# remydubois/illico

Hardware: NVIDIA B200
Metric: gene_x_group_tests_per_s (higher is better)
Workload: dtype f32 keys / int64 ranks / f64 epilogue

## Files before the change

illico_b200/csrc/fused.cu:

```cuda
#include "common.cuh"
#include "epilogue.cuh"
#include "tma.cuh"

#include <stdlib.h>

namespace illico {

int launch_stage_dense_list(const float* X, long long ld, int gene_lb, const int* list, const int* n_list_dev, const int* mode_dev,
                            int want_mode, const illico_plan_t* plan, float* ir_vals, uint32_t* ir_cnt, cudaStream_t stream);
int launch_stage_dense_tma_if(const float* X, long long ld, int gene_lb, int b, const illico_plan_t* plan, float* ir_vals,
                              uint32_t* ir_cnt, int seg_lo, int seg_hi, cudaStream_t stream, int segs_per_cta_req,
                              const int* mode_dev, int want_mode);
int launch_stage_csr_if(const float*, const int32_t*, const long long*, int, int, const illico_plan_t*, float*, uint32_t*, void*, size_t,
                        const int*, int, cudaStream_t);
int launch_stage_csr_list(const float*, const int32_t*, const long long*, int, int, const int*, const int*, int, int,
                          const illico_plan_t*, float*, uint32_t*, cudaStream_t);
int launch_ovo_mapped(const float*, const uint32_t*, int, const int*, const int*, int, const illico_plan_t*, const illico_flags_t*, double*,
                      long long, void*, size_t, const illico_debug_t*, cudaStream_t);
int launch_ovr_mapped(const float*, const uint32_t*, int, const int*, const int*, int, const illico_plan_t*, const illico_flags_t*, double*,
                      long long, void*, size_t, const illico_debug_t*, cudaStream_t);
bool stage_dense_tma_ok(const float* X, long long ld, int gene_lb, int b, const illico_plan_t* plan);
int launch_stage_dense_tma(const float* X, long long ld, int gene_lb, int b, const illico_plan_t* plan, float* ir_vals,
                           uint32_t* ir_cnt, int seg_lo, int seg_hi, cudaStream_t stream, int segs_per_cta = 0);

// ... 23 lines not shown
    double* gc;
    int Gs;
};
constexpr int DW = 64;
constexpr int CLS_NARROW = 1, CLS_IDENT = 2, CLS_WANTS_WIDE = 4;
constexpr int WIDE_FROM = 11;
constexpr int HB_NONE = 0, HB_LIST = 1, HB_ALL = 2;
constexpr int GC_MU = 0, GC_NRNT = 1, GC_PROD12 = 2, GC_DENOM = 3, GC_INV_NT = 4, GC_N = 5;

size_t gtab_bytes(int b, int G) {
    const size_t bs = (size_t)((b + 63) & ~63), Gs = (size_t)((G + 63) & ~63);
    return bs * ((size_t)DCAP * 20 + 4 + 8 + 8 + 1 + 8 + 2 + (size_t)DW * 2) + Gs * 8 * GC_N + 1024;
}
Gtab gtab_carve(void* ws, int b, int G) {
    const size_t bs = (size_t)((b + 63) & ~63), Gs = (size_t)((G + 63) & ~63);
    char* p = reinterpret_cast<char*>((reinterpret_cast<uintptr_t>(ws) + 255) & ~(uintptr_t)255);
    Gtab c;
    c.Gs = (int)Gs;
    c.gc = reinterpret_cast<double*>(p); p += Gs * 8 * GC_N;
    c.fval = reinterpret_cast<double*>(p); p += bs * 8 * DCAP;
    c.tie = reinterpret_cast<unsigned long long*>(p); p += bs * 8;
    c.sum = reinterpret_cast<double*>(p); p += bs * 8;
    c.key = reinterpret_cast<float*>(p); p += bs * 4 * DCAP;
    c.mult = reinterpret_cast<uint32_t*>(p); p += bs * 4 * DCAP;
    c.wgt = reinterpret_cast<uint32_t*>(p); p += bs * 4 * DCAP;
    c.nnz = reinterpret_cast<uint32_t*>(p); p += bs * 4;
    c.n_bad = reinterpret_cast<int*>(p); p += 64;
    c.list = reinterpret_cast<int*>(p); p += bs * 4;
    c.cmap = reinterpret_cast<int*>(p); p += bs * 4;
    c.wm = reinterpret_cast<uint32_t*>(p); p += bs * 2 * DW;
    c.bad = reinterpret_cast<unsigned char*>(p); p += bs;
    c.cls = reinterpret_cast<unsigned char*>(p); p += bs;
    c.mode = reinterpret_cast<unsigned char*>(p);
    return c;
}

constexpr float ROUND_MAGIC = 12582912.0f;
constexpr uint32_t ROUND_MAGIC_BITS = 0x4B400000u;
__device__ __forceinline__ uint32_t count_bin(float v, bool& ok) {
    const float tt = __fadd_rn(v, ROUND_MAGIC);
    const uint32_t q1 = __float_as_uint(tt) - (ROUND_MAGIC_BITS + 1u);
    ok = (__fsub_rn(tt, ROUND_MAGIC) == v) && (q1 < (uint32_t)DW);
    return q1;
}

__global__ void __launch_bounds__(256) fused_ctab_kernel(const float* __restrict__ ir_vals, const uint32_t* __restrict__ ir_cnt,
                                                         int b, const illico_plan_t pl, int seg_lo, int seg_hi, int is_log1p,
                                                         Gtab gt, int bs, int wide_on) {
    __shared__ uint32_t wh[8][DW];
    const int lane = threadIdx.x & 31, wl = threadIdx.x >> 5;
    const int warp = (blockIdx.x * blockDim.x + threadIdx.x) >> 5, nwarps = (gridDim.x * blockDim.x) >> 5;
    const int S = pl.n_segments;
    for (int j = warp; j < b; j += nwarps) {
        float mykey = 0.0f;
        uint32_t mycnt = 0;
        int D = 0;
        bool nbad = false;
        bool general = false;
        for (int s = seg_lo; s < seg_hi && !nbad; ++s) {
            const int c = (int)ir_cnt[(long long)j * S + s];
            const float* src = ir_vals + (long long)j * pl.slot_cap + pl.seg_base[s];
            for (int i0 = 0; i0 < c && !nbad; i0 += 32) {
                const bool valid = i0 + lane < c;
                const float v = valid ? src[i0 + lane] : 0.0f;
                if (__any_sync(FULL, valid && !(v > 0.0f))) { nbad = general = true; break; }
                const unsigned same = __match_any_sync(FULL, __float_as_uint(v));
                const bool leader = valid && (__ffs(same) - 1 == lane);
                const uint32_t n = (uint32_t)__popc(same);
                unsigned leaders = __ballot_sync(FULL, leader);
                while (leaders) {
                    const int l = __ffs(leaders) - 1;
                    leaders &= leaders - 1;
                    const float vv = __shfl_sync(FULL, v, l);
                    const uint32_t nn = __shfl_sync(FULL, n, l);
                    const unsigned hit = __ballot_sync(FULL, lane < D && mykey == vv);
                    if (hit) {
                        if (lane == __ffs(hit) - 1) mycnt += nn;
                    } else if (D < DCAP) {
                        if (lane == D) { mykey = vv; mycnt = nn; }
                        ++D;
                    } else {
                        nbad = true;
                        break;
                    }
                }
            }
        }
        bool ident = wide_on != 0 && !general;
        if (ident) {
            wh[wl][lane] = 0u;
            wh[wl][lane + 32] = 0u;
            __syncwarp();
            if (!nbad) {
                bool okv = true;
                const uint32_t q1 = count_bin(mykey, okv);
                if (__any_sync(FULL, lane < D && !okv)) ident = false;
                else if (lane < D) wh[wl][q1] = mycnt;
            } else {
                for (int s = seg_lo; s < seg_hi && ident; ++s) {
                    const int c = (int)ir_cnt[(long long)j * S + s];
                    const float* src = ir_vals + (long long)j * pl.slot_cap + pl.seg_base[s];
                    for (int i0 = 0; i0 < c; i0 += 32) {
                        const bool valid = i0 + lane < c;
                        const float v = valid ? src[i0 + lane] : 0.0f;
                        bool okv;
                        const uint32_t q1 = count_bin(v, okv);
                        if (__any_sync(FULL, valid && !okv)) { ident = false; break; }
                        const unsigned same = __match_any_sync(FULL, __float_as_uint(v));
                        if (valid && (__ffs(same) - 1 == lane)) wh[wl][q1] += (uint32_t)__popc(same);
                        __syncwarp();
                    }
                }
            }
            __syncwarp();
        }
        int cls = nbad ? 0 : CLS_NARROW;
        if (ident) {
            const uint32_t c0 = wh[wl][lane], c1 = wh[wl][lane + 32];
            if (__any_sync(FULL, (c0 | c1) > 0xffffu)) {
                ident = false;
            } else {
                const uint32_t e0 = wh[wl][2 * lane], e1 = wh[wl][2 * lane + 1];
                gt.wm[(long long)lane * bs + j] = e0 | (e1 << 16);
                cls |= CLS_IDENT;
                if (nbad || D >= WIDE_FROM) cls |= CLS_WANTS_WIDE;
            }
        }
        __syncwarp();
        if (lane == 0) gt.cls[j] = (unsigned char)cls;
        if (nbad) continue;
        int pos = 0;
        for (int t = 0; t < D; ++t) pos += (__shfl_sync(FULL, mykey, t) < mykey) ? 1 : 0;
        const bool mine = lane < D;
        if (mine) { gt.key[(long long)pos * bs + j] = mykey; gt.mult[(long long)pos * bs + j] = mycnt; }
        if (lane >= D && lane < DCAP) { gt.key[(long long)lane * bs + j] = 0.0f; gt.mult[(long long)lane * bs + j] = 0u; }
        const uint32_t nnz = warp_sum<uint32_t>(mine ? mycnt : 0u);
        const unsigned long long tie = warp_sum_u64(mine ? (unsigned long long)cube_minus((long long)mycnt) : 0ull);
        const double sum = warp_sum_f64(mine ? (double)mycnt * fc_value(mykey, is_log1p) : 0.0);
        if (lane == 0) { gt.nnz[j] = nnz; gt.tie[j] = tie; gt.sum[j] = sum; }
    }
}

__global__ void __launch_bounds__(256) fused_mode_kernel(int b, Gtab gt) {
    const int j = blockIdx.x * blockDim.x + threadIdx.x;
    const int c = (j < b) ? gt.cls[j] : 0;
    const bool tile_wide = __syncthreads_or((c & CLS_WANTS_WIDE) != 0) != 0;
    const int mode = (tile_wide && (c & CLS_IDENT)) ? 1 : 0;
    const bool bad = j < b && mode == 0 && !(c & CLS_NARROW);
    if (j < b) { gt.mode[j] = (unsigned char)mode; gt.bad[j] = bad ? 1 : 0; }
    const int nb = __syncthreads_count(bad);
    if (threadIdx.x == 0 && nb) atomicAdd(gt.n_bad, nb);
}

template <int ROWS, int STAGES, int BUF>
struct FusedLayout {
    static constexpr int ROW_BYTES = FUSED_LANES * 4;
    static constexpr int STAGE_BYTES = ROWS * ROW_BYTES;
    static constexpr int RING_OFF = 0;
    static constexpr int NZ_OFF = STAGES * STAGE_BYTES;
    static constexpr int KEY_OFF = NZ_OFF + BUF * ROW_BYTES;
    static constexpr int HIST_OFF = KEY_OFF + DCAP * ROW_BYTES;
    static constexpr int BAR_OFF = HIST_OFF + DCAP * FUSED_LANES * 2;
    static constexpr int BYTES = BAR_OFF + 2 * STAGES * 8;
};

template <int ROWS, int STAGES, int BUF, int MINB, bool OVO>
__global__ void __launch_bounds__(FUSED_THREADS, MINB) fused_pass_kernel(const float* __restrict__ X, long long ld, int gene_lb,
                                                                         int b, const illico_plan_t pl, int groups_per_cta,
                                                                         Gtab gt, int bs, unsigned long long* __restrict__ rec,
                                                                         long long gstride, int share_1024) {
    using L = FusedLayout<ROWS, STAGES, BUF>;
    static_assert(32 % ROWS == 0 && BUF > ROWS, "layout");
    extern __shared__ __align__(128) unsigned char smem[];
    const uint32_t smem_a = (uint32_t)__cvta_generic_to_shared(smem);
    const uint32_t bars = smem_a + L::BAR_OFF;
    const int t = threadIdx.x, lane = t & 31, w = t >> 5;
    const int G = pl.n_groups, ref = OVO ? pl.ref_group : -1;
    const int gy0 = blockIdx.y * groups_per_cta, gy1 = min(G, gy0 + groups_per_cta);
    const int p_begin = pl.seg_pos[pl.group_seg[gy0]], p_end = pl.seg_pos[pl.group_seg[gy1]];
    const bool ref_in = ref >= gy0 && ref < gy1;
    const int ref_p0 = ref_in ? pl.seg_pos[pl.group_seg[ref]] : 0;
    const int ref_len = ref_in ? pl.seg_pos[pl.group_seg[ref + 1]] - ref_p0 : 0;
    const int nv = p_end - p_begin - ref_len;
    const int g0 = blockIdx.x * FUSED_LANES;
    const uint32_t row_bytes = (uint32_t)min(FUSED_LANES, (b - g0 + 3) & ~3) * 4u;
    if (nv <= 0) return;
    if ((long long)gt.n_bad[0] * 1024 > (long long)b * share_1024) return;
    if (__syncthreads_and(t >= FUSED_LANES || g0 + t >= b || gt.bad[g0 + t] != 0 || gt.mode[g0 + t] != 0)) return;

    if (t == 0) {
        for (int i = 0; i < STAGES; ++i) {
            mbar_init(bars + 8 * i, 1);
            mbar_init(bars + 8 * (STAGES + i), FUSED_WARPS);
        }
        asm volatile("fence.mbarrier_init.release.cluster;" ::: "memory");
    }
    __syncthreads();

    if (w == FUSED_WARPS) {
        uint64_t policy;
        asm volatile("createpolicy.fractional.L2::evict_first.b64 %0, 1.0;" : "=l"(policy));
        const char* base = reinterpret_cast<const char*>(X + gene_lb + g0);
        const unsigned long long ldb = (unsigned long long)ld * 4ull;
        auto row_of = [&](int i) {
            int p = p_begin + i;
            if (ref_in && p >= ref_p0) p += ref_len;
            return pl.perm[p];
        };
        int myrow = (lane < nv) ? row_of(lane) : 0;
        int k = 0;
        for (int i0 = 0; i0 < nv; i0 += 32) {
            const int nxt = (i0 + 32 + lane < nv) ? row_of(i0 + 32 + lane) : 0;
            const int nrows = min(32, nv - i0);
#pragma unroll
            for (int q = 0; q < 32 / ROWS; ++q, ++k) {
                if (q * ROWS >= nrows) break;
                const int slot = k % STAGES;
                const uint32_t full = bars + 8 * slot, empty = bars + 8 * (STAGES + slot);
                mbar_wait(empty, ((k / STAGES) & 1) ^ 1);
                const int rows_here = min(ROWS, nrows - q * ROWS);
                if (lane == 0) mbar_expect_tx(full, (uint32_t)rows_here * row_bytes);
                __syncwarp();
                const int u = lane - q * ROWS;
                if (u >= 0 && u < rows_here)
                    bulk_g2s(smem_a + L::RING_OFF + slot * L::STAGE_BYTES + u * L::ROW_BYTES,
                             base + (unsigned long long)(uint32_t)myrow * ldb, row_bytes, full, policy);
            }
            myrow = nxt;
        }
        return;
    }

    const int j = g0 + t;
    const bool in_batch = j < b;
    const uint32_t keys_a = smem_a + L::KEY_OFF + t * 4;
    const uint32_t hist_a = smem_a + L::HIST_OFF + t * 2;
    const uint32_t nz_a = smem_a + L::NZ_OFF + t * 4;
    auto lds_f = [](uint32_t a) { float v; asm volatile("ld.shared.f32 %0, [%1];" : "=f"(v) : "r"(a)); return v; };
    auto sts_f = [](uint32_t a, float v) { asm volatile("st.shared.f32 [%0], %1;" ::"r"(a), "f"(v) : "memory"); };
    auto lds_h = [](uint32_t a) { uint16_t v; asm volatile("ld.shared.u16 %0, [%1];" : "=h"(v) : "r"(a)); return (uint32_t)v; };
    auto sts_h = [](uint32_t a, uint32_t v) { asm volatile("st.shared.u16 [%0], %1;" ::"r"(a), "h"((uint16_t)v) : "memory"); };
    const bool mine = in_batch && gt.bad[j] == 0 && gt.mode[j] == 0;
    bool bad = !mine;
    float* gkey = gt.key + (in_batch ? j : 0);
    int D = 0;
#pragma unroll
    for (int q = 0; q < DCAP; ++q) {
        const float kq = bad ? 0.0f : __ldcg(gkey + (long long)q * bs);
        if (kq != 0.0f) D = q + 1;
        sts_f(keys_a + q * L::ROW_BYTES, kq);
        sts_h(hist_a + q * (FUSED_LANES * 2), 0u);
    }
    uint32_t Hacc[OVO ? 1 : DCAP];
#pragma unroll
    for (int q = 0; q < (OVO ? 1 : DCAP); ++q) Hacc[q] = 0u;
    uint32_t wr = nz_a;

    auto drain = [&]() {
        const uint32_t mywr = bad ? nz_a : wr;
        const uint32_t maxwr = __reduce_max_sync(FULL, mywr - nz_a);
        for (uint32_t o = 0; o < maxwr; o += L::ROW_BYTES) {
            if (nz_a + o < mywr) {
                const float v = lds_f(nz_a + o);
                int q = (int)v - 1;
                if (!(q >= 0 && q < D && lds_f(keys_a + q * L::ROW_BYTES) == v)) {
                    q = 0;
                    while (q < D && lds_f(keys_a + q * L::ROW_BYTES) != v) ++q;
                    if (q == D) {
                        int slot = -1;
                        if (v > 0.0f) {
                            for (int r = D; r < DCAP && slot < 0; ++r) {
                                const unsigned old = atomicCAS(reinterpret_cast<unsigned*>(gkey + (long long)r * bs), 0u,
                                                               __float_as_uint(v));
                                const float kv = old ? __uint_as_float(old) : v;
                                sts_f(keys_a + r * L::ROW_BYTES, kv);
                                D = r + 1;
                                if (kv == v) slot = r;
                            }
                        }
                        if (slot < 0) { bad = true; q = 0; }
                        else q = slot;
                    }
                }
                const uint32_t ha = hist_a + q * (FUSED_LANES * 2);
                sts_h(ha, lds_h(ha) + 1u);
            }
        }
        wr = nz_a;
    };
    auto close_group = [&](int g) {
        drain();
        unsigned long long wds[3] = {0ull, 0ull, 0ull};
#pragma unroll
        for (int q = 0; q < DCAP; ++q) {
            const uint32_t bq = lds_h(hist_a + q * (FUSED_LANES * 2));
            wds[q >> 2] |= (unsigned long long)bq << (16 * (q & 3));
            if (!OVO) Hacc[OVO ? 0 : q] += bq;
            sts_h(hist_a + q * (FUSED_LANES * 2), 0u);
        }
        if (!bad) {
            unsigned long long* o = rec + (long long)g * gstride + (long long)j * 3;
            o[0] = wds[0]; o[1] = wds[1]; o[2] = wds[2];
        }
    };
    auto group_end_v = [&](int gg) { return pl.seg_pos[pl.group_seg[gg + 1]] - p_begin - ((ref_in && gg > ref) ? ref_len : 0); };
    int g = (gy0 == ref) ? gy0 + 1 : gy0;
    int gend = group_end_v(g);

    auto append = [&](float v) {
        asm volatile("{ .reg .pred p; setp.neu.f32 p, %1, 0f00000000; @p st.shared.f32 [%0], %1; @p add.u32 %0, %0, %2; }"
                     : "+r"(wr)
                     : "f"(v), "n"(L::ROW_BYTES)
                     : "memory");
    };
    const uint32_t ring_a = smem_a + L::RING_OFF + t * 4;
    const uint32_t wr_limit = nz_a + (uint32_t)(BUF - ROWS) * L::ROW_BYTES;
    int slot = 0;
    uint32_t parity = 0;
    for (int i = 0; i < nv; i += ROWS) {
        mbar_wait(bars + 8 * slot, parity);
        const uint32_t src = ring_a + slot * L::STAGE_BYTES;
        if (i + ROWS <= gend) {
            float v[ROWS];
#pragma unroll
            for (int u = 0; u < ROWS; ++u) v[u] = lds_f(src + u * L::ROW_BYTES);
#pragma unroll
            for (int u = 0; u < ROWS; ++u) append(v[u]);
        } else {
            const int nr = min(ROWS, nv - i);
#pragma unroll 1
            for (int u = 0; u < nr; ++u) {
                if (i + u == gend) {
                    close_group(g);
                    ++g;
                    if (g == ref) ++g;
                    gend = group_end_v(g);
                }
                append(lds_f(src + u * L::ROW_BYTES));
            }
        }
        __syncwarp();
        if (lane == 0) mbar_arrive(bars + 8 * (STAGES + slot));
        if (++slot == STAGES) { slot = 0; parity ^= 1u; }
        if (__any_sync(FULL, wr > wr_limit)) drain();
    }
    close_group(g);
    if (mine) {
        if (bad) {
            gt.bad[j] = 1;
        } else if (!OVO) {
#pragma unroll
            for (int q = 0; q < (OVO ? 1 : DCAP); ++q)
                if (Hacc[q]) atomicAdd(gt.mult + (long long)q * bs + j, Hacc[q]);
        }
    }
}

template <int ROWS, int STAGES>
struct WideLayout {
    static constexpr int ROW_BYTES = FUSED_LANES * 4;
    static constexpr int STAGE_BYTES = ROWS * ROW_BYTES;
    static constexpr int RING_OFF = 0;
    static constexpr int HIST_OFF = STAGES * STAGE_BYTES;
    static constexpr int ATAB_OFF = HIST_OFF + (DW / 2) * ROW_BYTES;
    static constexpr int BAR_OFF = ATAB_OFF + (DW / 2) * ROW_BYTES;
    static constexpr int BYTES = BAR_OFF + 2 * STAGES * 8;
};
constexpr int WIDE_M_SHIFT = 40;
static_assert(DW % 2 == 0 && DW <= 64, "packed layout: two 16-bit bins per word; the table step keeps two bins per lane");

template <int ROWS, int STAGES, int MINB>
__global__ void __launch_bounds__(FUSED_THREADS, MINB) fused_wide_pass_kernel(const float* __restrict__ X, long long ld, int gene_lb,
                                                                              int b, const illico_plan_t pl, int groups_per_cta,
                                                                              Gtab gt, int bs, unsigned long long* __restrict__ rec,
                                                                              long long gstride, int share_1024) {
    using L = WideLayout<ROWS, STAGES>;
    static_assert(32 % ROWS == 0, "layout");
    extern __shared__ __align__(128) unsigned char smem[];
    const uint32_t smem_a = (uint32_t)__cvta_generic_to_shared(smem);
    const uint32_t bars = smem_a + L::BAR_OFF;
    const int t = threadIdx.x, lane = t & 31, w = t >> 5;
    const int G = pl.n_groups, ref = pl.ref_group;
    const int g0 = blockIdx.x * FUSED_LANES;
    const uint32_t row_bytes = (uint32_t)min(FUSED_LANES, (b - g0 + 3) & ~3) * 4u;
    if ((long long)gt.n_bad[0] * 1024 > (long long)b * share_1024) return;
    if (__syncthreads_and(t >= FUSED_LANES || g0 + t >= b || gt.bad[g0 + t] != 0 || gt.mode[g0 + t] != 1)) return;

    if (t == 0) {
        for (int i = 0; i < STAGES; ++i) {
            mbar_init(bars + 8 * i, 1);
            mbar_init(bars + 8 * (STAGES + i), FUSED_WARPS);
        }
        asm volatile("fence.mbarrier_init.release.cluster;" ::: "memory");
    }
    __syncthreads();
    const int n_chunks = (G + groups_per_cta - 1) / groups_per_cta;
    struct Chunk { int gy0, p_begin, ref_p0, ref_len, nv; bool ref_in; };
    auto chunk_of = [&](int c) {
        Chunk k;
        k.gy0 = c * groups_per_cta;
        const int gy1 = min(G, k.gy0 + groups_per_cta);
        k.p_begin = pl.seg_pos[pl.group_seg[k.gy0]];
        const int p_end = pl.seg_pos[pl.group_seg[gy1]];
        k.ref_in = ref >= k.gy0 && ref < gy1;
        k.ref_p0 = k.ref_in ? pl.seg_pos[pl.group_seg[ref]] : 0;
        k.ref_len = k.ref_in ? pl.seg_pos[pl.group_seg[ref + 1]] - k.ref_p0 : 0;
        k.nv = p_end - k.p_begin - k.ref_len;
        return k;
    };

    if (w == FUSED_WARPS) {
        uint64_t policy;
        asm volatile("createpolicy.fractional.L2::evict_first.b64 %0, 1.0;" : "=l"(policy));
        const char* base = reinterpret_cast<const char*>(X + gene_lb + g0);
        const unsigned long long ldb = (unsigned long long)ld * 4ull;
        int k = 0;
        for (int c = blockIdx.y; c < n_chunks; c += gridDim.y) {
            const Chunk ch = chunk_of(c);
            auto row_of = [&](int i) {
                int p = ch.p_begin + i;
                if (ch.ref_in && p >= ch.ref_p0) p += ch.ref_len;
                return pl.perm[p];
            };
            int myrow = (lane < ch.nv) ? row_of(lane) : 0;
            for (int i0 = 0; i0 < ch.nv; i0 += 32) {
                const int nxt = (i0 + 32 + lane < ch.nv) ? row_of(i0 + 32 + lane) : 0;
                const int nrows = min(32, ch.nv - i0);
#pragma unroll
                for (int q = 0; q < 32 / ROWS; ++q, ++k) {
                    if (q * ROWS >= nrows) break;
                    const int slot = k % STAGES;
                    const uint32_t full = bars + 8 * slot, empty = bars + 8 * (STAGES + slot);
                    mbar_wait_backoff(empty, ((k / STAGES) & 1) ^ 1);
                    const int rows_here = min(ROWS, nrows - q * ROWS);
                    if (lane == 0) mbar_expect_tx(full, (uint32_t)rows_here * row_bytes);
                    __syncwarp();
                    const int u = lane - q * ROWS;
                    if (u >= 0 && u < rows_here)
                        bulk_g2s(smem_a + L::RING_OFF + slot * L::STAGE_BYTES + u * L::ROW_BYTES,
                                 base + (unsigned long long)(uint32_t)myrow * ldb, row_bytes, full, policy);
                }
                myrow = nxt;
            }
        }
        return;
    }

    const int j = g0 + t;
    const bool in_batch = j < b;
    const bool mine = in_batch && gt.bad[j] == 0 && gt.mode[j] == 1;
    const uint32_t hist_a = smem_a + L::HIST_OFF + (uint32_t)(w >> 1) * 128u + (uint32_t)lane * 4u + (uint32_t)(w & 1) * 2u;
    const uint32_t atab_a = smem_a + L::ATAB_OFF + t * 4;
    constexpr uint32_t BIN_BYTES = FUSED_LANES * 2;
    auto lds_f = [](uint32_t a) { float v; asm volatile("ld.shared.f32 %0, [%1];" : "=f"(v) : "r"(a)); return v; };
    auto lds_u = [](uint32_t a) { uint32_t v; asm volatile("ld.shared.u32 %0, [%1];" : "=r"(v) : "r"(a) : "memory"); return v; };
    auto sts_u = [](uint32_t a, uint32_t v) { asm volatile("st.shared.u32 [%0], %1;" ::"r"(a), "r"(v) : "memory"); };
    auto lds_h = [](uint32_t a) { uint32_t v; asm volatile("ld.shared.u16 %0, [%1];" : "=r"(v) : "r"(a) : "memory"); return v; };
    auto sts_h = [](uint32_t a, uint32_t v) { asm volatile("st.shared.u16 [%0], %1;" ::"r"(a), "r"(v) : "memory"); };
    {
        const uint32_t* wm_j = gt.wm + (in_batch ? j : 0);
#pragma unroll 8
        for (int q = 0; q < DW / 2; ++q) {
            sts_h(hist_a + (2 * q) * BIN_BYTES, 0u);
            sts_h(hist_a + (2 * q + 1) * BIN_BYTES, 0u);
            sts_u(atab_a + q * L::ROW_BYTES, mine ? __ldg(wm_j + (long long)q * bs) : 0u);
        }
    }
    bool bad = false;

    auto take = [&](float v) {
        bool ok;
        const uint32_t q1 = count_bin(v, ok);
        const uint32_t a = hist_a + q1 * BIN_BYTES;
        asm volatile(
            "{ .reg .pred p; .reg .u32 h;\n"
            "setp.ne.u32 p, %1, 0;\n"
            "@p ld.shared.u16 h, [%0];\n"
            "@p add.u32 h, h, 1;\n"
            "@p st.shared.u16 [%0], h; }"
            ::"r"(a), "r"((uint32_t)ok) : "memory");
        bad |= !ok && v != 0.0f;
    };
    auto close_group = [&](int g) {
        uint32_t m = 0, s1 = 0, above = 0;
        unsigned long long u2 = 0, tie = 0;
        auto bin = [&](uint32_t ha, uint32_t a, int q) {
            const uint32_t bq = lds_h(ha);
            if (bq) {
                sts_h(ha, 0u);
                u2 += (unsigned long long)bq * (2u * above + a);
                tie += (unsigned long long)(a * bq) * (3u * (a + bq));
                tie += (unsigned long long)(bq * bq) * bq;
                s1 += bq * (uint32_t)(q + 1);
                m += bq;
            }
            above += a;
        };
#pragma unroll 4
        for (int q = DW / 2 - 1; q >= 0; --q) {
            const uint32_t ab = lds_u(atab_a + q * L::ROW_BYTES);
            bin(hist_a + (2 * q + 1) * BIN_BYTES, ab >> 16, 2 * q + 1);
            bin(hist_a + (2 * q) * BIN_BYTES, ab & 0xffffu, 2 * q);
        }
        if (mine && !bad) {
            unsigned long long* o = rec + (long long)g * gstride + (long long)j * 3;
            o[0] = u2 | ((unsigned long long)m << WIDE_M_SHIFT);
            o[1] = tie - m;
// ... 359 lines not shown
                    const int jj = c[u] - c_lo;
                    int q = min(max((int)v[u] - 1, 0), DCAP - 1);
                    if (kq[u] != v[u]) q = gt.bad[j_lo + jj] ? -1 : gtab_slot(gt.key + j_lo + jj, bs, v[u]);
                    if (q >= 0) {
                        atomicAdd(&hist[jj * 6 + (q >> 1)], 1u << (16 * (q & 1)));
                    } else {
                        const int j = j_lo + jj;
                        const unsigned bit = 1u << (8 * (j & 3));
                        const unsigned old = atomicOr(reinterpret_cast<unsigned*>(gt.bad + (j & ~3)), bit);
                        if (!(old & bit)) atomicAdd(gt.n_bad, 1);
                    }
                }
            }
        }
    }
    __syncthreads();
    const bool multi = pl.group_seg[g + 1] - pl.group_seg[g] > 1;
    for (int jj = t; jj < ng; jj += CSRF_THREADS) {
        const int j = j_lo + jj;
        uint32_t wd[6];
#pragma unroll
        for (int k = 0; k < 6; ++k) wd[k] = hist[jj * 6 + k];
        if (OVO && g == pl.ref_group) {
#pragma unroll
            for (int q = 0; q < DCAP; ++q) {
                const uint32_t cq = (wd[q >> 1] >> (16 * (q & 1))) & 0xffffu;
                if (cq) atomicAdd(gt.mult + (long long)q * bs + j, cq);
            }
        } else if (!multi) {
            unsigned long long* o = rec + (long long)g * gstride + (long long)j * 3;
#pragma unroll
            for (int k = 0; k < 3; ++k) o[k] = (unsigned long long)wd[2 * k] | ((unsigned long long)wd[2 * k + 1] << 32);
        } else {
            uint32_t* o = reinterpret_cast<uint32_t*>(rec + (long long)g * gstride + (long long)j * 3);
#pragma unroll
            for (int k = 0; k < 6; ++k) if (wd[k]) atomicAdd(o + k, wd[k]);
        }
    }
}

__global__ void __launch_bounds__(256) fused_hist_sum_kernel(int b, int G, int groups_per_block, Gtab gt, int bs,
                                                             const unsigned long long* __restrict__ rec, long long gstride) {
    const int j = blockIdx.x * blockDim.x + threadIdx.x;
    if (j >= b || gt.bad[j]) return;
    const int ga = blockIdx.y * groups_per_block, gb = min(G, ga + groups_per_block);
    uint32_t acc[DCAP];
#pragma unroll
    for (int q = 0; q < DCAP; ++q) acc[q] = 0u;
    for (int g = ga; g < gb; ++g) {
        const unsigned long long* r = rec + (long long)g * gstride + (long long)j * 3;
        const unsigned long long wds[3] = {r[0], r[1], r[2]};
#pragma unroll
        for (int q = 0; q < DCAP; ++q) acc[q] += (uint32_t)((wds[q >> 2] >> (16 * (q & 3))) & 0xffffull);
    }
#pragma unroll
    for (int q = 0; q < DCAP; ++q)
        if (acc[q]) atomicAdd(gt.mult + (long long)q * bs + j, acc[q]);
}

__global__ void __launch_bounds__(1024) fused_list_kernel(int b, Gtab gt, int num, int den, int force_all) {
    __shared__ int wsum[32];
    __shared__ int base_s;
    const int t = threadIdx.x, lane = t & 31, w = t >> 5;
    if (t == 0) base_s = 0;
    __syncthreads();
    for (int j0 = 0; j0 < b; j0 += 1024) {
        const int j = j0 + t;
        const bool flag = j < b && gt.bad[j] != 0;
        const unsigned bal = __ballot_sync(FULL, flag);
        if (lane == 0) wsum[w] = __popc(bal);
        __syncthreads();
        int before = 0, total = 0;
        for (int ww = 0; ww < 32; ++ww) { const int c = wsum[ww]; if (ww < w) before += c; total += c; }
        const int base = base_s;
        if (j < b) {
            const int k = base + before + __popc(bal & ((1u << lane) - 1u));
            if (flag) gt.list[k] = j;
            gt.cmap[j] = flag ? k : -1;
        }
        __syncthreads();
        if (t == 0) base_s = base + total;
        __syncthreads();
    }
    const int n = base_s;
    const bool all = force_all || (long long)n * den > (long long)b * num;
    if (all && n > 0) {
        for (int j = t; j < b; j += 1024) { gt.list[j] = j; gt.cmap[j] = j; }
    }
    if (t == 0) {
        gt.n_bad[1] = (n == 0) ? 0 : (all ? b : n);
        gt.n_bad[2] = (n == 0) ? HB_NONE : (all ? HB_ALL : HB_LIST);
    }
}

int env_int(const char* name, int dflt) {
    const char* v = getenv(name);
    return v ? atoi(v) : dflt;
}
int list_share_1024() {
    const char* v = getenv("ILLICO_FUSED_LIST_SHARE");
    const double f = v ? atof(v) : 0.125;
    return (int)(f * 1024.0 + 0.5);
}

thread_local float g_last_fused_ms = -1.0f;

constexpr int PASS_ROWS = 1536;
constexpr int OVR_SAMPLE_CELLS = 16384;

template <bool OVO>
int run_fused(const float* X, long long ld, int gene_lb, int b, const illico_plan_t* plan, const illico_flags_t* flags,
              const illico_batch_buffers_t* buf, double* results, long long gstride, const illico_debug_t* dbg,
              cudaStream_t stream) {
    g_last_fused_ms = -1.0f;
    if (env_int(OVO ? "ILLICO_OVO_FUSED" : "ILLICO_OVR_FUSED", 1) == 0 || b <= 0) return -1;
    if (!stage_dense_tma_ok(X, ld, gene_lb, b, plan)) return -1;
    if (plan->max_target_group_size >= 65536 || plan->n_groups < 2 || plan->n_groups > 65535) return -1;
    if (OVO && (long long)plan->ref_group_size + plan->max_target_group_size > PAIR_MAX) return -1;
    if (!OVO && flags->group_sums) return -1;
    if (dbg) return -1;
    if (buf->workspace_bytes < gtab_bytes(b, plan->n_groups)) return -1;
    const int bs = (b + 63) & ~63;
    Gtab gt = gtab_carve(buf->workspace, b, plan->n_groups);

    const bool wide_on = OVO && !flags->is_log1p && env_int("ILLICO_FUSED_WIDE", 1) != 0;
    int seg_lo = plan->ref_seg_begin, seg_hi = plan->ref_seg_end;
    if (!OVO) {
        long long avg = plan->n_cells / plan->n_segments;
        if (avg < 1) avg = 1;
        seg_lo = 0;
        seg_hi = (int)((OVR_SAMPLE_CELLS + avg - 1) / avg);
        if (seg_hi < 1) seg_hi = 1;
        if (seg_hi > plan->n_segments) seg_hi = plan->n_segments;
    }
    ILLICO_CUDA_OK(cudaMemsetAsync(gt.n_bad, 0, 16 * sizeof(int), stream));
    {
        const int rc = launch_stage_dense_tma(X, ld, gene_lb, b, plan, buf->ir_vals, buf->ir_cnt, seg_lo, seg_hi, stream, 1);
        if (rc != 0) return rc;
        int blocks = (b + 7) / 8;
        if (blocks > 148 * 8) blocks = 148 * 8;
        ILLICO_LAUNCH("fused_ctab_kernel", stream, fused_ctab_kernel<<<blocks, 256, 0, stream>>>(buf->ir_vals, buf->ir_cnt, b, *plan, seg_lo, seg_hi, flags->is_log1p, gt, bs, wide_on ? 1 : 0));
        ILLICO_LAUNCH("fused_mode_kernel", stream, fused_mode_kernel<<<(b + FUSED_LANES - 1) / FUSED_LANES, FUSED_LANES, 0, stream>>>(b, gt));
        ILLICO_CUDA_OK(cudaGetLastError());
    }
    if (!OVO)
        ILLICO_CUDA_OK(cudaMemsetAsync(gt.mult, 0, (size_t)bs * DCAP * sizeof(uint32_t), stream));

    long long avg_g = plan->n_cells / plan->n_groups;
    if (avg_g < 1) avg_g = 1;
    int gpc = (int)(PASS_ROWS / avg_g);
    if (gpc < 1) gpc = 1;
    {
        using L = FusedLayout<8, 5, 16>;
        auto kern = fused_pass_kernel<8, 5, 16, 3, OVO>;
        ILLICO_CUDA_OK(cudaFuncSetAttribute(kern, cudaFuncAttributeMaxDynamicSharedMemorySize, (int)L::BYTES));
        const dim3 grid((unsigned)((b + FUSED_LANES - 1) / FUSED_LANES), (unsigned)((plan->n_groups + gpc - 1) / gpc));
        ILLICO_LAUNCH("fused_pass_kernel", stream, kern<<<grid, FUSED_THREADS, L::BYTES, stream>>>(X, ld, gene_lb, b, *plan, gpc, gt, bs,
                                                        reinterpret_cast<unsigned long long*>(results), gstride, list_share_1024()));
        ILLICO_CUDA_OK(cudaGetLastError());
    }
    if (wide_on) {
        auto kern = fused_wide_pass_kernel<8, 5, 2>;
        const int wide_smem = WideLayout<8, 5>::BYTES;
        ILLICO_CUDA_OK(cudaFuncSetAttribute(kern, cudaFuncAttributeMaxDynamicSharedMemorySize, wide_smem));
        const int tiles = (b + FUSED_LANES - 1) / FUSED_LANES, chunks = (plan->n_groups + gpc - 1) / gpc;
        int gy = (2 * 148) / tiles;
        if (gy < 1) gy = 1;
        if (gy > chunks) gy = chunks;
        const dim3 grid((unsigned)tiles, (unsigned)gy);
        ILLICO_LAUNCH("fused_wide_pass_kernel", stream, kern<<<grid, FUSED_THREADS, wide_smem, stream>>>(
                X, ld, gene_lb, b, *plan, gpc, gt, bs, reinterpret_cast<unsigned long long*>(results), gstride, list_share_1024()));
        ILLICO_CUDA_OK(cudaGetLastError());
    }
    g_last_fused_ms = 0.0f;

    ILLICO_LAUNCH("fused_group_kernel", stream, fused_group_kernel<OVO><<<(plan->n_groups + 255) / 256, 256, 0, stream>>>(*plan, gt));
    ILLICO_LAUNCH("fused_gene_kernel", stream, fused_gene_kernel<OVO><<<(b + 127) / 128, 128, 0, stream>>>(b, *plan, *flags, gt, bs, nullptr, nullptr));
    ILLICO_CUDA_OK(cudaGetLastError());
    const bool score = flags->scores != nullptr;
    auto epi = score ? fused_epilogue_kernel<OVO, false, true> : fused_epilogue_kernel<OVO, false, false>;
    ILLICO_LAUNCH("fused_epilogue_kernel", stream, epi<<<dim3((unsigned)((b + 255) / 256), (unsigned)((plan->n_groups + EPI_GROUPS - 1) / EPI_GROUPS)), 256, 0, stream>>>(
            b, *plan, *flags, gt, bs, results, gstride, nullptr, nullptr, nullptr, list_share_1024()));
    if (wide_on) {
        auto wepi = score ? fused_epilogue_kernel<OVO, true, true> : fused_epilogue_kernel<OVO, true, false>;
        ILLICO_LAUNCH("fused_wide_epilogue_kernel", stream, wepi<<<dim3((unsigned)((b + 255) / 256), (unsigned)((plan->n_groups + EPI_GROUPS - 1) / EPI_GROUPS)), 256, 0, stream>>>(
                b, *plan, *flags, gt, bs, results, gstride, nullptr, nullptr, nullptr, list_share_1024()));
    }
    ILLICO_CUDA_OK(cudaGetLastError());

    ILLICO_LAUNCH("fused_list_kernel", stream, fused_list_kernel<<<1, 1024, 0, stream>>>(b, gt, list_share_1024(), 1024, 0));
    ILLICO_CUDA_OK(cudaGetLastError());
    if (launch_stage_dense_list(X, ld, gene_lb, gt.list, gt.n_bad + 1, gt.n_bad + 2, HB_LIST, plan, buf->ir_vals, buf->ir_cnt, stream))
        return 1;
    if (launch_stage_dense_tma_if(X, ld, gene_lb, b, plan, buf->ir_vals, buf->ir_cnt, 0, plan->n_segments, stream, 0, gt.n_bad + 2,
                                  HB_ALL))
        return 1;
    const size_t tab = (gtab_bytes(b, plan->n_groups) + 255) & ~(size_t)255;
    if (buf->workspace_bytes <= tab) return 1;
    char* ws = reinterpret_cast<char*>(buf->workspace) + tab;
    const size_t ws_bytes = buf->workspace_bytes - tab;
    return OVO ? launch_ovo_mapped(buf->ir_vals, buf->ir_cnt, b, gt.n_bad + 1, gt.list, b, plan, flags, results, gstride, ws, ws_bytes,
                                   nullptr, stream)
               : launch_ovr_mapped(buf->ir_vals, buf->ir_cnt, b, gt.n_bad + 1, gt.list, b, plan, flags, results, gstride, ws, ws_bytes,
                                   nullptr, stream);
}

}

float ovo_fused_last_ms() { return g_last_fused_ms; }

size_t ovo_fused_workspace_bytes(int b, int n_groups) { return gtab_bytes(b, n_groups); }

int launch_ovo_dense_fused(const float* X, long long ld, int gene_lb, int b, const illico_plan_t* plan,
                           const illico_flags_t* flags, const illico_batch_buffers_t* buf, double* results, long long gstride,
                           const illico_debug_t* dbg, cudaStream_t stream) {
    return run_fused<true>(X, ld, gene_lb, b, plan, flags, buf, results, gstride, dbg, stream);
}

int launch_ovr_dense_fused(const float* X, long long ld, int gene_lb, int b, const illico_plan_t* plan,
                           const illico_flags_t* flags, const illico_batch_buffers_t* buf, double* results, long long gstride,
                           const illico_debug_t* dbg, cudaStream_t stream) {
    return run_fused<false>(X, ld, gene_lb, b, plan, flags, buf, results, gstride, dbg, stream);
}


namespace {

template <bool OVO>
int run_fused_csr(const float* data, const int32_t* indices, const long long* indptr, int gene_lb, int b,
                  const illico_plan_t* plan, const illico_flags_t* flags, const illico_batch_buffers_t* buf, double* results,
                  long long gstride, const illico_debug_t* dbg, cudaStream_t stream) {
    g_last_fused_ms = -1.0f;
    if (env_int(OVO ? "ILLICO_OVO_FUSED" : "ILLICO_OVR_FUSED", 1) == 0 || env_int("ILLICO_CSR_FUSED", 1) == 0 || b <= 0) return -1;
    if (plan->max_target_group_size >= 65536 || plan->n_groups < 2 || plan->n_groups > 65535 || plan->n_segments > 65535) return -1;
    if (OVO && (long long)plan->ref_group_size + plan->max_target_group_size > PAIR_MAX) return -1;
    if (!OVO && flags->group_sums) return -1;
    if (dbg) return -1;
    if (buf->workspace_bytes < gtab_bytes(b, plan->n_groups)) return -1;
    const int bs = (b + 63) & ~63;
    Gtab gt = gtab_carve(buf->workspace, b, plan->n_groups);
    unsigned long long* rec = reinterpret_cast<unsigned long long*>(results);
    const int G = plan->n_groups;

    ILLICO_CUDA_OK(cudaMemsetAsync(gt.n_bad, 0, 16 * sizeof(int), stream));
    ILLICO_LAUNCH("fused_seed_kernel", stream, fused_seed_kernel<<<(bs + 255) / 256, 256, 0, stream>>>(gt, bs, flags->is_log1p ? 0 : 1));
    ILLICO_LAUNCH("fused_zero_multi_kernel", stream, fused_zero_multi_kernel<<<dim3(8, (unsigned)G), 256, 0, stream>>>(b, *plan, rec, gstride));
    ILLICO_CUDA_OK(cudaGetLastError());
    {
        auto kern = fused_csr_pass_kernel<OVO>;
        const int tile = b < CSRF_TILE ? b : CSRF_TILE;
        const size_t smem = (size_t)tile * 24;
        ILLICO_CUDA_OK(cudaFuncSetAttribute(kern, cudaFuncAttributeMaxDynamicSharedMemorySize, (int)smem));
        const dim3 grid((unsigned)((b + CSRF_TILE - 1) / CSRF_TILE), (unsigned)plan->n_segments);
        ILLICO_LAUNCH("fused_csr_pass_kernel", stream, kern<<<grid, CSRF_THREADS, smem, stream>>>(data, indices, indptr, gene_lb, b, *plan, gt, bs, rec, gstride));
        ILLICO_CUDA_OK(cudaGetLastError());
    }
    g_last_fused_ms = 0.0f;
    if (!OVO) {
        const int gpb = 64;
        ILLICO_LAUNCH("fused_hist_sum_kernel", stream, fused_hist_sum_kernel<<<dim3((unsigned)((b + 255) / 256), (unsigned)((G + gpb - 1) / gpb)), 256, 0, stream>>>(b, G, gpb, gt, bs, rec,
                                                                                                                 gstride));
    }
    ILLICO_LAUNCH("fused_group_kernel", stream, fused_group_kernel<OVO><<<(plan->n_groups + 255) / 256, 256, 0, stream>>>(*plan, gt));
    ILLICO_LAUNCH("fused_gene_kernel", stream, fused_gene_kernel<OVO><<<(b + 127) / 128, 128, 0, stream>>>(b, *plan, *flags, gt, bs, nullptr, nullptr));
    auto epi = flags->scores ? fused_epilogue_kernel<OVO, false, true> : fused_epilogue_kernel<OVO, false, false>;
    ILLICO_LAUNCH("fused_epilogue_kernel", stream, epi<<<dim3((unsigned)((b + 255) / 256), (unsigned)((G + EPI_GROUPS - 1) / EPI_GROUPS)), 256, 0, stream>>>(
            b, *plan, *flags, gt, bs, results, gstride, nullptr, nullptr, nullptr, 128));
    ILLICO_CUDA_OK(cudaGetLastError());

    int share = list_share_1024();
    if (share > 128) share = 128;
    ILLICO_LAUNCH("fused_list_kernel", stream, fused_list_kernel<<<1, 1024, 0, stream>>>(b, gt, share, 1024, 0));
    ILLICO_CUDA_OK(cudaGetLastError());
    const size_t tab = (gtab_bytes(b, plan->n_groups) + 255) & ~(size_t)255;
    if (buf->workspace_bytes <= tab) return 1;
    char* ws = reinterpret_cast<char*>(buf->workspace) + tab;
    const size_t ws_bytes = buf->workspace_bytes - tab;
    const int max_list = (int)(((long long)b * share) / 1024) + 1;
    if (launch_stage_csr_list(data, indices, indptr, gene_lb, b, gt.cmap, gt.n_bad + 2, HB_LIST, max_list < b ? max_list : b, plan,
                              buf->ir_vals, buf->ir_cnt, stream)) return 1;
    if (launch_stage_csr_if(data, indices, indptr, gene_lb, b, plan, buf->ir_vals, buf->ir_cnt, ws, ws_bytes, gt.n_bad + 2, HB_ALL, stream))
        return 1;
    return OVO ? launch_ovo_mapped(buf->ir_vals, buf->ir_cnt, b, gt.n_bad + 1, gt.list, b, plan, flags, results, gstride, ws, ws_bytes,
                                   nullptr, stream)
               : launch_ovr_mapped(buf->ir_vals, buf->ir_cnt, b, gt.n_bad + 1, gt.list, b, plan, flags, results, gstride, ws, ws_bytes,
                                   nullptr, stream);
}

}

int launch_ovo_csr_fused(const float* data, const int32_t* indices, const long long* indptr, int gene_lb, int b,
                         const illico_plan_t* plan, const illico_flags_t* flags, const illico_batch_buffers_t* buf, double* results,
                         long long gstride, const illico_debug_t* dbg, cudaStream_t stream) {
    return run_fused_csr<true>(data, indices, indptr, gene_lb, b, plan, flags, buf, results, gstride, dbg, stream);
}
int launch_ovr_csr_fused(const float* data, const int32_t* indices, const long long* indptr, int gene_lb, int b,
                         const illico_plan_t* plan, const illico_flags_t* flags, const illico_batch_buffers_t* buf, double* results,
                         long long gstride, const illico_debug_t* dbg, cudaStream_t stream) {
    return run_fused_csr<false>(data, indices, indptr, gene_lb, b, plan, flags, buf, results, gstride, dbg, stream);
}

}
```

Measured before the change: 7.066 billion.

## Make fused pass kernel persistent with atomic work-stealing over tile×group-chunk items

The fused pass kernel becomes a persistent kernel with a grid of about 3 CTAs per SM. Its producer warp pulls (gene tile, group chunk) work items from a global atomic counter and hands each item's metadata and group boundaries to the consumer warps. The handoff goes through a double-buffered shared-memory queue guarded by mbarriers. This replaces the one-CTA-per-item launch, aiming to cut launch and tail imbalance and the cost of CTAs that exit early. In exchange it adds atomic contention, per-item synchronization, and a cap of 96 groups per chunk; it also reuses a slot in n_bad as the counter, which must be reset before each launch.

Result: no change. 7.004 billion (median of 6 runs) (-0.9%).

```diff
diff --git a/illico_b200/csrc/fused.cu b/illico_b200/csrc/fused.cu
--- a/illico_b200/csrc/fused.cu
+++ b/illico_b200/csrc/fused.cu
@@ -199,6 +199,8 @@
     if (threadIdx.x == 0 && nb) atomicAdd(gt.n_bad, nb);
 }
 
+constexpr int ITEM_GROUPS = 96;
+constexpr int ITEM_INTS = 4 + ITEM_GROUPS;
 template <int ROWS, int STAGES, int BUF>
 struct FusedLayout {
     static constexpr int ROW_BYTES = FUSED_LANES * 4;
@@ -207,8 +209,9 @@
     static constexpr int NZ_OFF = STAGES * STAGE_BYTES;
     static constexpr int KEY_OFF = NZ_OFF + BUF * ROW_BYTES;
     static constexpr int HIST_OFF = KEY_OFF + DCAP * ROW_BYTES;
-    static constexpr int BAR_OFF = HIST_OFF + DCAP * FUSED_LANES * 2;
-    static constexpr int BYTES = BAR_OFF + 2 * STAGES * 8;
+    static constexpr int ITEM_OFF = HIST_OFF + DCAP * FUSED_LANES * 2;
+    static constexpr int BAR_OFF = ITEM_OFF + 2 * ITEM_INTS * 4;
+    static constexpr int BYTES = BAR_OFF + 2 * (STAGES + 2) * 8;
 };
 
 template <int ROWS, int STAGES, int BUF, int MINB, bool OVO>
@@ -217,69 +220,108 @@
                                                                          Gtab gt, int bs, unsigned long long* __restrict__ rec,
                                                                          long long gstride, int share_1024) {
     using L = FusedLayout<ROWS, STAGES, BUF>;
-    static_assert(32 % ROWS == 0 && BUF > ROWS, "layout");
+    static_assert(32 % ROWS == 0 && BUF > ROWS && ITEM_GROUPS % 32 == 0, "layout");
     extern __shared__ __align__(128) unsigned char smem[];
     const uint32_t smem_a = (uint32_t)__cvta_generic_to_shared(smem);
-    const uint32_t bars = smem_a + L::BAR_OFF;
+    const uint32_t bars = smem_a + L::BAR_OFF, qbars = bars + 16 * STAGES;
+    const uint32_t item_a = smem_a + L::ITEM_OFF;
     const int t = threadIdx.x, lane = t & 31, w = t >> 5;
     const int G = pl.n_groups, ref = OVO ? pl.ref_group : -1;
-    const int gy0 = blockIdx.y * groups_per_cta, gy1 = min(G, gy0 + groups_per_cta);
-    const int p_begin = pl.seg_pos[pl.group_seg[gy0]], p_end = pl.seg_pos[pl.group_seg[gy1]];
-    const bool ref_in = ref >= gy0 && ref < gy1;
-    const int ref_p0 = ref_in ? pl.seg_pos[pl.group_seg[ref]] : 0;
-    const int ref_len = ref_in ? pl.seg_pos[pl.group_seg[ref + 1]] - ref_p0 : 0;
-    const int nv = p_end - p_begin - ref_len;
-    const int g0 = blockIdx.x * FUSED_LANES;
-    const uint32_t row_bytes = (uint32_t)min(FUSED_LANES, (b - g0 + 3) & ~3) * 4u;
-    if (nv <= 0) return;
+    const int tiles = (b + FUSED_LANES - 1) / FUSED_LANES;
+    const int n_items = tiles * ((G + groups_per_cta - 1) / groups_per_cta);
     if ((long long)gt.n_bad[0] * 1024 > (long long)b * share_1024) return;
-    if (__syncthreads_and(t >= FUSED_LANES || g0 + t >= b || gt.bad[g0 + t] != 0 || gt.mode[g0 + t] != 0)) return;
 
     if (t == 0) {
         for (int i = 0; i < STAGES; ++i) {
             mbar_init(bars + 8 * i, 1);
             mbar_init(bars + 8 * (STAGES + i), FUSED_WARPS);
         }
+        for (int e = 0; e < 2; ++e) {
+            mbar_init(qbars + 8 * e, 1);
+            mbar_init(qbars + 16 + 8 * e, FUSED_WARPS);
+        }
         asm volatile("fence.mbarrier_init.release.cluster;" ::: "memory");
     }
     __syncthreads();
+    auto sts_i = [](uint32_t a, int v) { asm volatile("st.shared.s32 [%0], %1;" ::"r"(a), "r"(v) : "memory"); };
+    auto lds_i = [](uint32_t a) { int v; asm volatile("ld.shared.s32 %0, [%1];" : "=r"(v) : "r"(a) : "memory"); return v; };
 
     if (w == FUSED_WARPS) {
         uint64_t policy;
         asm volatile("createpolicy.fractional.L2::evict_first.b64 %0, 1.0;" : "=l"(policy));
-        const char* base = reinterpret_cast<const char*>(X + gene_lb + g0);
         const unsigned long long ldb = (unsigned long long)ld * 4ull;
-        auto row_of = [&](int i) {
-            int p = p_begin + i;
-            if (ref_in && p >= ref_p0) p += ref_len;
-            return pl.perm[p];
-        };
-        int myrow = (lane < nv) ? row_of(lane) : 0;
-        int k = 0;
-        for (int i0 = 0; i0 < nv; i0 += 32) {
-            const int nxt = (i0 + 32 + lane < nv) ? row_of(i0 + 32 + lane) : 0;
-            const int nrows = min(32, nv - i0);
-#pragma unroll
-            for (int q = 0; q < 32 / ROWS; ++q, ++k) {
-                if (q * ROWS >= nrows) break;
-                const int slot = k % STAGES;
-                const uint32_t full = bars + 8 * slot, empty = bars + 8 * (STAGES + slot);
-                mbar_wait(empty, ((k / STAGES) & 1) ^ 1);
-                const int rows_here = min(ROWS, nrows - q * ROWS);
-                if (lane == 0) mbar_expect_tx(full, (uint32_t)rows_here * row_bytes);
+        int k = 0, n = 0;
+        int it = blockIdx.x;
+        while (it < n_items) {
+            int nx = 0;
+            if (lane == 0) nx = atomicAdd(gt.n_bad + 3, 1) + (int)gridDim.x;
+            const int tile = it % tiles, c = it / tiles;
+            const int g0 = tile * FUSED_LANES;
+            bool any = false;
+#pragma unroll
+            for (int e = 0; e < FUSED_LANES / 32; ++e) {
+                const int jj = g0 + 32 * e + lane;
+                any |= jj < b && gt.bad[jj] == 0 && gt.mode[jj] == 0;
+            }
+            const int gy0 = c * groups_per_cta, gy1 = min(G, gy0 + groups_per_cta);
+            const int p_begin = pl.seg_pos[pl.group_seg[gy0]], p_end = pl.seg_pos[pl.group_seg[gy1]];
+            const bool ref_in = ref >= gy0 && ref < gy1;
+            const int ref_p0 = ref_in ? pl.seg_pos[pl.group_seg[ref]] : 0;
+            const int ref_len = ref_in ? pl.seg_pos[pl.group_seg[ref + 1]] - ref_p0 : 0;
+            const int nv = p_end - p_begin - ref_len;
+            int ends[ITEM_GROUPS / 32];
+#pragma unroll
+            for (int r = 0; r < ITEM_GROUPS / 32; ++r) {
+                const int gg = gy0 + 32 * r + lane;
+                ends[r] = (gg < gy1) ? pl.seg_pos[pl.group_seg[gg + 1]] - p_begin - ((ref_in && gg > ref) ? ref_len : 0) : 0;
+            }
+            auto row_of = [&](int i) {
+                int p = p_begin + i;
+                if (ref_in && p >= ref_p0) p += ref_len;
+                return pl.perm[p];
+            };
+            if (__any_sync(FULL, any) && nv > 0) {
+                int myrow = (lane < nv) ? row_of(lane) : 0;
+                const int e = n & 1;
+                const uint32_t ia = item_a + e * (ITEM_INTS * 4);
+                mbar_wait(qbars + 16 + 8 * e, ((n >> 1) & 1) ^ 1);
+                if (lane == 0) { sts_i(ia, tile); sts_i(ia + 4, nv); sts_i(ia + 8, gy0); }
+#pragma unroll
+                for (int r = 0; r < ITEM_GROUPS / 32; ++r)
+                    if (gy0 + 32 * r + lane < gy1) sts_i(ia + 16 + 4 * (32 * r + lane), ends[r]);
                 __syncwarp();
-                const int u = lane - q * ROWS;
-                if (u >= 0 && u < rows_here)
-                    bulk_g2s(smem_a + L::RING_OFF + slot * L::STAGE_BYTES + u * L::ROW_BYTES,
-                             base + (unsigned long long)(uint32_t)myrow * ldb, row_bytes, full, policy);
-            }
-            myrow = nxt;
-        }
+                if (lane == 0) mbar_arrive(qbars + 8 * e);
+                ++n;
+                const char* base = reinterpret_cast<const char*>(X + gene_lb + g0);
+                const uint32_t row_bytes = (uint32_t)min(FUSED_LANES, (b - g0 + 3) & ~3) * 4u;
+                for (int i0 = 0; i0 < nv; i0 += 32) {
+                    const int nxt = (i0 + 32 + lane < nv) ? row_of(i0 + 32 + lane) : 0;
+                    const int nrows = min(32, nv - i0);
+#pragma unroll
+                    for (int q = 0; q < 32 / ROWS; ++q, ++k) {
+                        if (q * ROWS >= nrows) break;
+                        const int slot = k % STAGES;
+                        const uint32_t full = bars + 8 * slot, empty = bars + 8 * (STAGES + slot);
+                        mbar_wait(empty, ((k / STAGES) & 1) ^ 1);
+                        const int rows_here = min(ROWS, nrows - q * ROWS);
+                        if (lane == 0) mbar_expect_tx(full, (uint32_t)rows_here * row_bytes);
+                        __syncwarp();
+                        const int u = lane - q * ROWS;
+                        if (u >= 0 && u < rows_here)
+                            bulk_g2s(smem_a + L::RING_OFF + slot * L::STAGE_BYTES + u * L::ROW_BYTES,
+                                     base + (unsigned long long)(uint32_t)myrow * ldb, row_bytes, full, policy);
+                    }
+                    myrow = nxt;
+                }
+            }
+            it = __shfl_sync(FULL, nx, 0);
+        }
+        const int e = n & 1;
+        mbar_wait(qbars + 16 + 8 * e, ((n >> 1) & 1) ^ 1);
+        if (lane == 0) { sts_i(item_a + e * (ITEM_INTS * 4), -1); mbar_arrive(qbars + 8 * e); }
         return;
     }
 
-    const int j = g0 + t;
-    const bool in_batch = j < b;
     const uint32_t keys_a = smem_a + L::KEY_OFF + t * 4;
     const uint32_t hist_a = smem_a + L::HIST_OFF + t * 2;
     const uint32_t nz_a = smem_a + L::NZ_OFF + t * 4;
@@ -287,17 +329,10 @@
     auto sts_f = [](uint32_t a, float v) { asm volatile("st.shared.f32 [%0], %1;" ::"r"(a), "f"(v) : "memory"); };
     auto lds_h = [](uint32_t a) { uint16_t v; asm volatile("ld.shared.u16 %0, [%1];" : "=h"(v) : "r"(a)); return (uint32_t)v; };
     auto sts_h = [](uint32_t a, uint32_t v) { asm volatile("st.shared.u16 [%0], %1;" ::"r"(a), "h"((uint16_t)v) : "memory"); };
-    const bool mine = in_batch && gt.bad[j] == 0 && gt.mode[j] == 0;
-    bool bad = !mine;
-    float* gkey = gt.key + (in_batch ? j : 0);
+    int tile = -1, j = 0;
+    bool mine = false, bad = true;
+    float* gkey = gt.key;
     int D = 0;
-#pragma unroll
-    for (int q = 0; q < DCAP; ++q) {
-        const float kq = bad ? 0.0f : __ldcg(gkey + (long long)q * bs);
-        if (kq != 0.0f) D = q + 1;
-        sts_f(keys_a + q * L::ROW_BYTES, kq);
-        sts_h(hist_a + q * (FUSED_LANES * 2), 0u);
-    }
     uint32_t Hacc[OVO ? 1 : DCAP];
 #pragma unroll
     for (int q = 0; q < (OVO ? 1 : DCAP); ++q) Hacc[q] = 0u;
@@ -350,10 +385,19 @@
             o[0] = wds[0]; o[1] = wds[1]; o[2] = wds[2];
         }
     };
-    auto group_end_v = [&](int gg) { return pl.seg_pos[pl.group_seg[gg + 1]] - p_begin - ((ref_in && gg > ref) ? ref_len : 0); };
-    int g = (gy0 == ref) ? gy0 + 1 : gy0;
-    int gend = group_end_v(g);
-
+    auto finish_tile = [&]() {
+        if (mine) {
+            if (bad) {
+                gt.bad[j] = 1;
+            } else if (!OVO) {
+#pragma unroll
+                for (int q = 0; q < (OVO ? 1 : DCAP); ++q)
+                    if (Hacc[q]) atomicAdd(gt.mult + (long long)q * bs + j, Hacc[q]);
+            }
+        }
+#pragma unroll
+        for (int q = 0; q < (OVO ? 1 : DCAP); ++q) Hacc[q] = 0u;
+    };
     auto append = [&](float v) {
         asm volatile("{ .reg .pred p; setp.neu.f32 p, %1, 0f00000000; @p st.shared.f32 [%0], %1; @p add.u32 %0, %0, %2; }"
                      : "+r"(wr)
@@ -364,42 +408,63 @@
     const uint32_t wr_limit = nz_a + (uint32_t)(BUF - ROWS) * L::ROW_BYTES;
     int slot = 0;
     uint32_t parity = 0;
-    for (int i = 0; i < nv; i += ROWS) {
-        mbar_wait(bars + 8 * slot, parity);
-        const uint32_t src = ring_a + slot * L::STAGE_BYTES;
-        if (i + ROWS <= gend) {
-            float v[ROWS];
-#pragma unroll
-            for (int u = 0; u < ROWS; ++u) v[u] = lds_f(src + u * L::ROW_BYTES);
-#pragma unroll
-            for (int u = 0; u < ROWS; ++u) append(v[u]);
-        } else {
-            const int nr = min(ROWS, nv - i);
+    for (int n = 0;; ++n) {
+        const int e = n & 1;
+        const uint32_t ia = item_a + e * (ITEM_INTS * 4);
+        mbar_wait(qbars + 8 * e, (n >> 1) & 1);
+        const int x = lds_i(ia);
+        if (x != tile && tile >= 0) finish_tile();
+        if (x < 0) break;
+        if (x != tile) {
+            tile = x;
+            j = tile * FUSED_LANES + t;
+            const bool in_batch = j < b;
+            mine = in_batch && gt.bad[j] == 0 && gt.mode[j] == 0;
+            bad = !mine;
+            gkey = gt.key + (in_batch ? j : 0);
+            D = 0;
+#pragma unroll
+            for (int q = 0; q < DCAP; ++q) {
+                const float kq = bad ? 0.0f : __ldcg(gkey + (long long)q * bs);
+                if (kq != 0.0f) D = q + 1;
+                sts_f(keys_a + q * L::ROW_BYTES, kq);
+                sts_h(hist_a + q * (FUSED_LANES * 2), 0u);
+            }
+        }
+        const int nv = lds_i(ia + 4), gy0 = lds_i(ia + 8);
+        const uint32_t ends_a = ia + 16 - 4 * gy0;
+        int g = (gy0 == ref) ? gy0 + 1 : gy0;
+        int gend = lds_i(ends_a + 4 * g);
+        for (int i = 0; i < nv; i += ROWS) {
+            mbar_wait(bars + 8 * slot, parity);
+            const uint32_t src = ring_a + slot * L::STAGE_BYTES;
+            if (i + ROWS <= gend) {
+                float v[ROWS];
+#pragma unroll
+                for (int u = 0; u < ROWS; ++u) v[u] = lds_f(src + u * L::ROW_BYTES);
+#pragma unroll
+                for (int u = 0; u < ROWS; ++u) append(v[u]);
+            } else {
+                const int nr = min(ROWS, nv - i);
 #pragma unroll 1
-            for (int u = 0; u < nr; ++u) {
-                if (i + u == gend) {
-                    close_group(g);
-                    ++g;
-                    if (g == ref) ++g;
-                    gend = group_end_v(g);
+                for (int u = 0; u < nr; ++u) {
+                    if (i + u == gend) {
+                        close_group(g);
+                        ++g;
+                        if (g == ref) ++g;
+                        gend = lds_i(ends_a + 4 * g);
+                    }
+                    append(lds_f(src + u * L::ROW_BYTES));
                 }
-                append(lds_f(src + u * L::ROW_BYTES));
-            }
-        }
+            }
+            __syncwarp();
+            if (lane == 0) mbar_arrive(bars + 8 * (STAGES + slot));
+            if (++slot == STAGES) { slot = 0; parity ^= 1u; }
+            if (__any_sync(FULL, wr > wr_limit)) drain();
+        }
+        close_group(g);
         __syncwarp();
-        if (lane == 0) mbar_arrive(bars + 8 * (STAGES + slot));
-        if (++slot == STAGES) { slot = 0; parity ^= 1u; }
-        if (__any_sync(FULL, wr > wr_limit)) drain();
-    }
-    close_group(g);
-    if (mine) {
-        if (bad) {
-            gt.bad[j] = 1;
-        } else if (!OVO) {
-#pragma unroll
-            for (int q = 0; q < (OVO ? 1 : DCAP); ++q)
-                if (Hacc[q]) atomicAdd(gt.mult + (long long)q * bs + j, Hacc[q]);
-        }
+        if (lane == 0) mbar_arrive(qbars + 16 + 8 * e);
     }
 }
 
@@ -1065,10 +1130,16 @@
     if (gpc < 1) gpc = 1;
     {
         using L = FusedLayout<8, 5, 16>;
+        static_assert(3 * (L::BYTES + 1024) <= 228 * 1024, "3 CTAs per SM: 228 KB of shared memory per SM, 1 KB reserved per CTA");
         auto kern = fused_pass_kernel<8, 5, 16, 3, OVO>;
         ILLICO_CUDA_OK(cudaFuncSetAttribute(kern, cudaFuncAttributeMaxDynamicSharedMemorySize, (int)L::BYTES));
-        const dim3 grid((unsigned)((b + FUSED_LANES - 1) / FUSED_LANES), (unsigned)((plan->n_groups + gpc - 1) / gpc));
-        ILLICO_LAUNCH("fused_pass_kernel", stream, kern<<<grid, FUSED_THREADS, L::BYTES, stream>>>(X, ld, gene_lb, b, *plan, gpc, gt, bs,
+        int dev = 0, sms = 0;
+        ILLICO_CUDA_OK(cudaGetDevice(&dev));
+        ILLICO_CUDA_OK(cudaDeviceGetAttribute(&sms, cudaDevAttrMultiProcessorCount, dev));
+        const int gpc_n = gpc < ITEM_GROUPS ? gpc : ITEM_GROUPS;
+        const long long items = (long long)((b + FUSED_LANES - 1) / FUSED_LANES) * ((plan->n_groups + gpc_n - 1) / gpc_n);
+        const int grid = (int)(items < 3LL * sms ? items : 3LL * sms);
+        ILLICO_LAUNCH("fused_pass_kernel", stream, kern<<<grid, FUSED_THREADS, L::BYTES, stream>>>(X, ld, gene_lb, b, *plan, gpc_n, gt, bs,
                                                         reinterpret_cast<unsigned long long*>(results), gstride, list_share_1024()));
         ILLICO_CUDA_OK(cudaGetLastError());
     }
```
